# lightdock/lightdock-rust

Measured on AMD Instinct MI355X. Metric: pose-energy evals/sec (DFIRE, 1k4c), higher is better.
Workload: dtype f64; 1 GPU; 1k4c DFIRE pose-energy batch, 8192 poses/GPU/step, 3413 x 3268 atoms, synthetic DCparams; parallelism=swarm-sharded x1, no collectives, nominal_pair_tests_per_pose=11153684

## Files before the change

### lightdock-rust_amd/csrc/kernels/dfire_bm.hip

```cpp
#include "dfire_bm.hpp"

#include <algorithm>
#include <cmath>
#include <cstddef>
#include <cstdlib>
#include <type_traits>

#include "dfire_device.hpp"
#include "dfire_bm_batch.inc"

#if !defined(LD_DIAG_BUILD) && (defined(LD_BM_DIAG_ANM_COST) || defined(LD_BM_DIAG_ANM_LDS) || defined(LD_BM_DIAG_FIRST) || defined(LD_BM_DIAG_NO_ATOMIC) || defined(LD_BM_DIAG_NO_DMA) || defined(LD_BM_DIAG_NO_EXACT) || defined(LD_BM_DIAG_NO_EXACT_ATOMIC) || defined(LD_BM_DIAG_NO_PAIRS) || defined(LD_BM_DIAG_NO_PARTIAL) || defined(LD_BM_DIAG_NO_POSE) || defined(LD_BM_DIAG_NO_TRACKED) || defined(LD_BM_DIAG_ROW_OF_LANE) || defined(LD_BM_DIAG_WAIT) || defined(LD_BM_DIAG_CULL_TIMES) || defined(LD_BM_DIAG_NO_TP_ATOMIC))
#error "LD_BM_DIAG_* needs -DLD_DIAG_BUILD (tools/build_variant.sh)"
#endif

namespace ld {

namespace {

typedef const __attribute__((address_space(4))) BmLaunch BmArgs;
#define LD_BM_ARGS ((BmArgs *)__builtin_amdgcn_kernarg_segment_ptr())

#ifndef LD_BM_CULL_POSES
#define LD_BM_CULL_POSES 8
#endif
// ... 637 lines not shown
        }
        T->job_count[3] = at;
    }
    __syncthreads();
    for (uint32_t base = 0; base < n_jobs; base += 8 * kStep) {
        uint32_t cost[8];
#pragma unroll
        for (int u = 0; u < 8; u++) {
            const uint32_t j = base + (uint32_t)u * kStep + (uint32_t)tid;
            cost[u] = j < n_jobs ? T->job_cost[j] : 0u;
        }
#pragma unroll
        for (int u = 0; u < 8; u++)
            if (cost[u]) T->job_order[atomicAdd(&s_class[class_of(cost[u])], 1u)] = base + (uint32_t)u * kStep + (uint32_t)tid;
    }
}

template <bool ANM>
struct BmWaveSharedT {
    static constexpr int kPart = ANM ? kBmAnmPartEntries : kBmPartEntries;
    unsigned char row_bits[kPart];
    unsigned short items[kPart + 64];
    alignas(16) float modes[ANM ? 2 * kBmModeFloats : 4];
};
template <bool ANM>
struct BmSharedT {
    unsigned char lut[kBmLutBytes];
    unsigned char cube[kBmWaves][kBmCubeBytes];
    BmWaveSharedT<ANM> w[kBmWaves];
};
typedef BmSharedT<false> BmShared;
static_assert(sizeof(BmSharedT<false>) * kBmGroupsPerCu <= 160 * 1024 && sizeof(BmSharedT<true>) * kBmGroupsPerCu <= 160 * 1024, "two workgroups per CU");
static_assert(offsetof(BmShared, cube) + sizeof(unsigned char[kBmWaves][kBmCubeBytes]) < 65536, "cube rows are addressed by instruction offsets");
static_assert(offsetof(BmSharedT<true>, cube) == offsetof(BmShared, cube), "one batch code for both forms");

struct BmWaveCtx {
    size_t tp;
    int ls;
    int RT;
    size_t lo;
};

#ifndef LD_BM_DRAIN_AT
#define LD_BM_DRAIN_AT 256
#endif
#ifndef LD_BM_EXACT_U
#define LD_BM_EXACT_U 4
#endif
constexpr int kBmDrainAt = LD_BM_DRAIN_AT;
__device__ __forceinline__ unsigned long long bm_pair_item(uint32_t row, int la, int ra) {
    return (unsigned long long)row | (unsigned long long)la << 32 | (unsigned long long)ra << 48;
}

__device__ __forceinline__ void bm_exact_pairs(BmArgs *T, unsigned long long *queue, uint32_t n_pairs, int lane) {
#ifdef LD_BM_DIAG_NO_EXACT
    return;
#endif
    __builtin_amdgcn_fence(__ATOMIC_RELEASE, "workgroup");
    constexpr int U = LD_BM_EXACT_U;
    const ExactCtx ex0 = bm_exact_ctx(T, 0);
    const size_t flag_words = (size_t)(T->m.rec_flag_words + T->m.lig.flag_words);
    for (uint32_t base = 0; base < n_pairs; base += 64 * U) {
        unsigned long long item[U];
        bool act[U];
        int la[U], ra[U];
        size_t row[U], pose[U];
#pragma unroll
        for (int u = 0; u < U; u++) {
            const uint32_t k = base + (uint32_t)(u * 64 + lane);
            act[u] = k < n_pairs;
            item[u] = act[u] ? __hip_atomic_load(queue + k, __ATOMIC_RELAXED, __HIP_MEMORY_SCOPE_AGENT) : 0ull;
        }
#pragma unroll
        for (int u = 0; u < U; u++) {
            la[u] = (int)((item[u] >> 32) & 0xffffu);
            ra[u] = (int)(item[u] >> 48);
            act[u] = act[u] && la[u] < T->m.lig.n_real && ra[u] < T->m.rec_n_real;
            row[u] = (size_t)(item[u] & 0xffffffffull);
        }
        typedef double v2d __attribute__((ext_vector_type(2)));
        v2d pq[U][4], lq[U][2], rq[U][2];
#pragma unroll
        for (int u = 0; u < U; u++) {
            const v2d *prow = reinterpret_cast<const v2d *>(T->rt_exact + (act[u] ? row[u] : 0) * 8);
            const v2d *lrow = reinterpret_cast<const v2d *>(T->m.lig_exact + (size_t)(act[u] ? la[u] : 0) * 4);
            const v2d *rrow = reinterpret_cast<const v2d *>(T->m.rec_exact + (size_t)(act[u] ? ra[u] : 0) * 4);
#pragma unroll
            for (int c = 0; c < 4; c++) pq[u][c] = prow[c];
            lq[u][0] = lrow[0]; lq[u][1] = lrow[1];
            rq[u][0] = rrow[0]; rq[u][1] = rrow[1];
        }
        double pr[U][7], lc[U][3], rc[U][3];
        uint32_t lterm[U], rterm[U];
        int32_t rslot[U], lslot[U];
#pragma unroll
        for (int u = 0; u < U; u++) {
            pr[u][0] = pq[u][0].x; pr[u][1] = pq[u][0].y; pr[u][2] = pq[u][1].x; pr[u][3] = pq[u][1].y;
            pr[u][4] = pq[u][2].x; pr[u][5] = pq[u][2].y; pr[u][6] = pq[u][3].x;
            pose[u] = (size_t)__double_as_longlong(pq[u][3].y);
            lc[u][0] = lq[u][0].x; lc[u][1] = lq[u][0].y; lc[u][2] = lq[u][1].x;
            rc[u][0] = rq[u][0].x; rc[u][1] = rq[u][0].y; rc[u][2] = rq[u][1].x;
            const unsigned long long lw = (unsigned long long)__double_as_longlong(lq[u][1].y), rw = (unsigned long long)__double_as_longlong(rq[u][1].y);
            lterm[u] = (uint32_t)lw; lslot[u] = (int32_t)(lw >> 32);
            rterm[u] = (uint32_t)rw; rslot[u] = (int32_t)(rw >> 32);
        }
        bool inside[U];
        uint32_t slot_at[U];
#pragma unroll
        for (int u = 0; u < U; u++) {
            inside[u] = false;
            slot_at[u] = 0u;
            if (!act[u]) continue;
            if (T->exact_pairs) atomicAdd(T->exact_pairs + row[u], 1u);
            const Quat q{pr[u][3], pr[u][4], pr[u][5], pr[u][6]};
            const Quat r = qmul(qmul(q, Quat{0.0, lc[u][0], lc[u][1], lc[u][2]}), qinverse(q));
            double px = r.x + pr[u][0], py = r.y + pr[u][1], pz = r.z + pr[u][2];
            double rx = rc[u][0], ry = rc[u][1], rz = rc[u][2];
            if (T->amp != nullptr) {
                const v2d *amps = reinterpret_cast<const v2d *>(T->amp_exact + row[u] * (2 * kBmMaxModes));
                const v2d *lm = reinterpret_cast<const v2d *>(T->m.lig_modes_exact + (size_t)la[u] * (3 * kBmMaxModes));
                const v2d *rm = reinterpret_cast<const v2d *>(T->m.rec_modes_exact + (size_t)ra[u] * (3 * kBmMaxModes));
#pragma unroll
                for (int k2 = 0; k2 < kBmMaxModes / 2; k2++) {
                    if (2 * k2 < T->m.anm_lig) {
                        const v2d c = amps[kBmMaxModes / 2 + k2], m0 = lm[3 * k2], m1 = lm[3 * k2 + 1], m2 = lm[3 * k2 + 2];
                        px += m0.x * c.x; py += m0.y * c.x; pz += m1.x * c.x;
                        if (2 * k2 + 1 < T->m.anm_lig) { px += m1.y * c.y; py += m2.x * c.y; pz += m2.y * c.y; }
                    }
                    if (2 * k2 < T->m.anm_rec) {
                        const v2d c = amps[k2], m0 = rm[3 * k2], m1 = rm[3 * k2 + 1], m2 = rm[3 * k2 + 2];
                        rx += m0.x * c.x; ry += m0.y * c.x; rz += m1.x * c.x;
                        if (2 * k2 + 1 < T->m.anm_rec) { rx += m1.y * c.y; ry += m2.x * c.y; rz += m2.y * c.y; }
                    }
                }
            }
            const double dx = 2.0 * rx - 2.0 * px, dy = 2.0 * ry - 2.0 * py, dz = 2.0 * rz - 2.0 * pz;
            const double D = dx * dx + dy * dy + dz * dz;
            if (!(D <= kCutScaled)) continue;
            uint32_t bin = 0;
            for (int b = 1; b <= 20; b++) bin += D >= ex0.step4[b] ? 1u : 0u;
            if (D <= ex0.iface_scaled) {
                uint32_t *flags = T->flags + pose[u] * flag_words;
                if (rslot[u] >= 0) atomicOr(&flags[rslot[u] >> 5], 1u << (rslot[u] & 31));
                if (lslot[u] >= 0) atomicOr(&flags[T->m.rec_flag_words + (lslot[u] >> 5)], 1u << (lslot[u] & 31));
            }
            inside[u] = true;
            slot_at[u] = (lterm[u] + rterm[u] + tiled_bin_term(bin)) / 8u;
        }
        double value[U];
#pragma unroll
        for (int u = 0; u < U; u++) value[u] = ex0.table[slot_at[u]];
#pragma unroll
        for (int u = 0; u < U; u++) {
            if (!inside[u]) continue;
            const long long fix = T->count_mode ? 1ll : __double2ll_rn(value[u] * T->m.fix_scale);
#ifndef LD_BM_DIAG_NO_EXACT_ATOMIC
            if (fix != 0) atomicAdd(reinterpret_cast<unsigned long long *>(T->exact_fix + row[u]), (unsigned long long)fix);
#else
            asm volatile("" :: "v"(fix));
#endif
        }
    }
    __builtin_amdgcn_fence(__ATOMIC_ACQ_REL, "workgroup");
}

__device__ __forceinline__ uint32_t bm_cell(float Rs, float Rz, float Ry, float Rx, float l2, float lz, float ly, float lx) {
    float D = Rs - l2;
    D = __builtin_fmaf(Rz, lz, D);
    D = __builtin_fmaf(Ry, ly, D);
    D = __builtin_fmaf(Rx, lx, D);
    uint32_t c;
    asm("v_cvt_u32_f32 %0, %1" : "=v"(c) : "v"(D));
    return c;
}

__device__ __forceinline__ unsigned long long bm_block_item(size_t entry, int a, int b) {
    return (unsigned long long)entry | (unsigned long long)a << 32 | (unsigned long long)b << 35;
}
__device__ __forceinline__ uint32_t bm_recheck(BmArgs *T, const unsigned char *lut, const unsigned long long *blocks, uint32_t n_blocks,
                                            unsigned long long *queue, uint32_t n_pairs, int lane) {
    __builtin_amdgcn_fence(__ATOMIC_RELEASE, "workgroup");
    constexpr float seed = (float)kBmCellZero + 0.5f;
    const int n_rt = T->m.rec_n_tiles;
    for (uint32_t base = 0; base < n_blocks; base += 64) {
    if (n_pairs > (uint32_t)kBmQueuePairs - 4096u - (uint32_t)(8 * kBmPartEntries)) {
        bm_exact_pairs(T, queue, n_pairs, lane);
        n_pairs = 0;
    }
    const bool act = base + (uint32_t)lane < n_blocks;
    const unsigned long long item = act ? __hip_atomic_load(blocks + base + lane, __ATOMIC_RELAXED, __HIP_MEMORY_SCOPE_AGENT) : 0ull;
    const size_t entry = (size_t)(item & 0xffffffffull);
    const int a = (int)((item >> 32) & 7u), b = (int)((item >> 35) & 7u);
    const size_t tp = entry / T->cap;
    const int lt = (int)(tp / (unsigned)n_rt), RT = (int)(tp % (unsigned)n_rt), ls = lt * 8 + a;
    const uint32_t row = act ? T->ent_row[entry] : 0u;
    const float4 *ap = reinterpret_cast<const float4 *>(T->rt) + (size_t)row * 3;
    const float4 a0 = ap[0], a1 = ap[1], a2 = ap[2];
    const TiledBox box = T->m.rec_sub[(size_t)RT * 8 + b];
    const float cbx = 0.5f * (box.lox + box.hix), cby = 0.5f * (box.loy + box.hiy), cbz = 0.5f * (box.loz + box.hiz);
    const Affine A{a0.x, a0.y, a0.z, a0.w - cbx, a1.x, a1.y, a1.z, a1.w - cby, a2.x, a2.y, a2.z, a2.w - cbz};
    const bool anm = T->amp != nullptr;
    float amp_rec[kBmMaxModes], amp_lig[kBmMaxModes];
    bool wild = false;
#pragma unroll
    for (int k = 0; k < kBmMaxModes; k++) amp_rec[k] = amp_lig[k] = 0.f;
    if (anm) {
        const float *am = T->amp + (size_t)row * kBmAmpFloats;
#pragma unroll
        for (int k = 0; k < kBmMaxModes; k++) {
            amp_rec[k] = am[k];
            amp_lig[k] = am[kBmMaxModes + k];
        }
        wild = am[20] != 0.f;
    }
    auto flexed = [&](const float *modes, const float *amps, int atom, int c) {
        const float *m = modes + ((atom >> 1) * 3 + c) * kBmMaxModes * 2 + (atom & 1);
        float d = amps[0] * m[0];
#pragma unroll
        for (int k = 1; k < kBmMaxModes; k++) d = __builtin_fmaf(amps[k], m[2 * k], d);
        return d;
    };
    float lx[8], ly[8], lz[8], l2[8];
#pragma unroll
    for (int i = 0; i < 8; i++) {
        const float4 L = reinterpret_cast<const float4 *>(T->m.lig_local)[ls * 8 + i];
        bm_apply(A, L.x, L.y, L.z, lx[i], ly[i], lz[i]);
        if (anm) {
            const float *lm = T->m.lig_modes_f32 + (size_t)ls * kBmModeFloats;
            lx[i] += flexed(lm, amp_lig, i, 0);
            ly[i] += flexed(lm, amp_lig, i, 1);
            lz[i] += flexed(lm, amp_lig, i, 2);
        }
        l2[i] = __builtin_fmaf(lx[i], lx[i], __builtin_fmaf(ly[i], ly[i], lz[i] * lz[i]));
    }
    const float *rec = reinterpret_cast<const float *>(T->m.rec_pairs + (size_t)RT * 32 + b * 4);
    const uint32_t near_code = T->m.lig_sub_tracked[ls] != 0 || T->m.rec_sub_tracked[RT * 8 + b] != 0 ? bm_code_of_bin(1) : 0xffffffffu;
#pragma unroll 1
    for (int q = 0; q < 4; q++) {
#pragma unroll
        for (int h = 0; h < 2; h++) {
            float x = rec[q * 8 + h] - cbx, y = rec[q * 8 + 2 + h] - cby, z = rec[q * 8 + 4 + h] - cbz;
            if (anm) {
                const float *rm = T->m.rec_modes_f32 + ((size_t)RT * 8 + (size_t)b) * kBmModeFloats;
                x += flexed(rm, amp_rec, 2 * q + h, 0);
                y += flexed(rm, amp_rec, 2 * q + h, 1);
                z += flexed(rm, amp_rec, 2 * q + h, 2);
            }
            const float Rs = __builtin_fmaf(-x, x, __builtin_fmaf(-y, y, __builtin_fmaf(-z, z, seed)));
            const float Rx = x * 2.f, Ry = y * 2.f, Rz = z * 2.f;
#pragma unroll
            for (int i = 0; i < 8; i++) {
                const uint32_t cell = bm_cell(Rs, Rz, Ry, Rx, l2[i], lz[i], ly[i], lx[i]);
                const uint32_t code = lut[cell];
                const bool hit = act && (wild || code == kBmFlagged || (near_code != 0xffffffffu && code <= near_code));
                const unsigned long long m = __builtin_amdgcn_ballot_w64(hit);
                if (hit) {
                    const uint32_t at = n_pairs + __builtin_amdgcn_mbcnt_hi((uint32_t)(m >> 32), __builtin_amdgcn_mbcnt_lo((uint32_t)m, 0u));
                    queue[at] = bm_pair_item(row, ls * 8 + i, RT * 64 + b * 8 + 2 * q + h);
                }
                n_pairs += (uint32_t)__popcll(m);
            }
        }
    }
    }
    return n_pairs;
}

template <bool DEBUG, bool ANM>
__global__ __launch_bounds__(kBmWaves * 64, kBmGroupsPerCu) void dfire_bm_pairs(const BmLaunch launch_arguments) {
    BmArgs *T = LD_BM_ARGS;
    __shared__ __attribute__((aligned(16))) BmSharedT<ANM> S;
    static_assert(offsetof(BmShared, lut) == 0, "the LUT's cell is its LDS address");
    static_assert(kBmWaves * kBmGroupsPerCu == 8, "dfire_bm_batch.inc clobbers v220..v255: 256 VGPRs a wave = two waves per SIMD");
    if ((uint32_t)(uintptr_t)&S != 0u) __builtin_trap();
    const int tid = threadIdx.x, lane = tid & 63;
    const int wave = __builtin_amdgcn_readfirstlane(tid >> 6);
    const int n_rt = T->m.rec_n_tiles;
    if (T->job_count[3] == 0) return;
    {
        const uint8_t *lut = T->count_mode ? T->m.lut_full : T->m.lut;
        for (int i = tid; i < kBmLutBytes / 16; i += kBmWaves * 64) reinterpret_cast<uint4 *>(S.lut)[i] = reinterpret_cast<const uint4 *>(lut)[i];
    }
    BmWaveSharedT<ANM> &WS = S.w[wave];
    __syncthreads();
    const uint32_t n_jobs = T->job_count[3];
    unsigned long long *queue = T->queue + ((size_t)blockIdx.x * kBmWaves + wave) * kBmQueueCap;
    unsigned long long *queue_blocks = queue + kBmQueuePairs;
    uint32_t queued = 0, queued_blocks = 0;
    const unsigned char *table_rows = reinterpret_cast<const unsigned char *>(T->count_mode ? T->m.rows_ones : T->m.rows);
    const unsigned long long dbg_t0 = DEBUG ? __builtin_amdgcn_s_memrealtime() : 0ull;
    unsigned long long dbg_jobs = 0, dbg_batches = 0, dbg_t_batch = 0, dbg_t_drain = 0, dbg_t_scan = 0, dbg_t_block = 0;
    unsigned long long dbg_t_dma = 0, dbg_t_compact = 0, dbg_t_compact_read = 0, dbg_t_chain = 0, dbg_t_wait = 0, dbg_blocks = 0;
    auto now = [] { return DEBUG ? __builtin_amdgcn_s_memrealtime() : 0ull; };

    const uint32_t n_waves = gridDim.x * (uint32_t)kBmWaves;
    bool first_job = true;
    for (;;) {
        const unsigned long long dbg_tj = now();
        uint32_t job = blockIdx.x * (uint32_t)kBmWaves + (uint32_t)wave;
        if (!first_job) {
            if (lane == 0) job = atomicAdd(T->job_next, 1u);
            job = (uint32_t)__builtin_amdgcn_readfirstlane((int)job) + n_waves;
        }
        first_job = false;
        if (job >= n_jobs) break;
        job = T->job_order[job];
        const uint4 rec = reinterpret_cast<const uint4 *>(T->job_rec)[job];
        const size_t tp = (size_t)(uint32_t)__builtin_amdgcn_readfirstlane((int)rec.x);
        const uint32_t lo = (uint32_t)__builtin_amdgcn_readfirstlane((int)rec.y), hi = (uint32_t)__builtin_amdgcn_readfirstlane((int)rec.z);
        const int a = __builtin_amdgcn_readfirstlane((int)rec.w);
        const int lt = (int)(tp / (unsigned)n_rt), RT = (int)(tp % (unsigned)n_rt);
        const int ls = lt * 8 + a;

        const uint32_t roff_all = T->m.rec_rowoff[(size_t)RT * 64 + lane];
        uint32_t any_bits = 0;
        {
            constexpr int kChunks = BmWaveSharedT<ANM>::kPart / 64;
            const unsigned long long *mask_at = T->ent_mask + (tp * T->cap + lo + (size_t)lane);
            unsigned long long m[kChunks];
#pragma unroll
            for (int k = 0; k < kChunks; k++) m[k] = mask_at[k * 64];
            const uint32_t n_mine = hi - lo;
#pragma unroll
            for (int k = 0; k < kChunks; k++) {
                const uint32_t bits = (uint32_t)(k * 64 + lane) < n_mine ? (uint32_t)(m[k] >> (8 * a)) & 0xffu : 0u;
                WS.row_bits[k * 64 + lane] = (unsigned char)bits;
                any_bits |= bits;
            }
        }
#pragma unroll
        for (int off = 32; off > 0; off >>= 1) any_bits |= (uint32_t)__shfl_xor((int)any_bits, off, 64);
        any_bits = (uint32_t)__builtin_amdgcn_readfirstlane((int)any_bits);
        if (any_bits == 0) continue;
        if (DEBUG) dbg_jobs++;

        v2f LocX[4], LocY[4], LocZ[4];
        {
            const float mine = T->m.lig_local[(size_t)(ls * 8 + (lane & 7)) * 4 + (lane < 24 ? lane >> 3 : 0)];
            auto from = [&](int l) { return __int_as_float(__builtin_amdgcn_readlane(__float_as_int(mine), l)); };
#pragma unroll
            for (int p2 = 0; p2 < 4; p2++) {
                LocX[p2] = v2f{from(2 * p2), from(2 * p2 + 1)};
                LocY[p2] = v2f{from(8 + 2 * p2), from(9 + 2 * p2)};
                LocZ[p2] = v2f{from(16 + 2 * p2), from(17 + 2 * p2)};
            }
        }
        if (ANM) {
            __builtin_amdgcn_fence(__ATOMIC_ACQ_REL, "wavefront");
            if (lane < kBmModeFloats / 4) reinterpret_cast<float4 *>(WS.modes)[lane] = reinterpret_cast<const float4 *>(T->m.lig_modes_f32 + (size_t)ls * kBmModeFloats)[lane];
        }
        constexpr int kRowPieces = kBmRowBytes / 16, kDmaRows = 64 / kRowPieces, kDma = (kBmCubeRows + kDmaRows - 1) / kDmaRows;
        static_assert(kRowPieces == 11 && kDmaRows == 5 && kDma == 13, "five rows per copy");
        const bool lig_tracked = T->m.lig_sub_tracked[ls] != 0;
        const uint32_t my_tracked = T->m.rec_sub_tracked[RT * 8 + (lane & 7)];
        const uint32_t lig_rowbase = T->m.lig_rowbase[ls * 8 + (lane & 7)];
        long long *const my_partial = T->ent_partial + ((size_t)blockIdx.x * kBmWaves + wave) * kBmPartEntries;
        const size_t row_base_entry = tp * T->cap + lo;
        const uint32_t *const job_rows = T->ent_row + row_base_entry;
// ... 220 lines not shown
                        const uint32_t lds_at = (uint32_t)(uintptr_t)&WS.items[0];
                        asm volatile(".rept 30\n\t"
                                     "ds_read_b128 v[220:223], %6\n\tds_read_b128 v[224:227], %6 offset:16\n\tds_read_b128 v[228:231], %6 offset:32\n\tds_read_b128 v[232:235], %6 offset:48\n\t"
                                     "s_waitcnt lgkmcnt(0)\n\t"
                                     "v_pk_fma_f32 %0, %4, v[220:221], %0\n\tv_pk_fma_f32 %1, %4, v[222:223], %1\n\tv_pk_fma_f32 %2, %5, v[224:225], %2\n\tv_pk_fma_f32 %3, %5, v[226:227], %3\n\t"
                                     "v_pk_fma_f32 %0, %4, v[228:229], %0\n\tv_pk_fma_f32 %1, %4, v[230:231], %1\n\tv_pk_fma_f32 %2, %5, v[232:233], %2\n\tv_pk_fma_f32 %3, %5, v[234:235], %3\n\t"
                                     ".endr\n\t"
                                     ".rept 9\n\tv_pk_fma_f32 %0, %4, %5, %0\n\tv_pk_fma_f32 %1, %4, %5, %1\n\tv_pk_fma_f32 %2, %4, %5, %2\n\tv_pk_fma_f32 %3, %4, %5, %3\n\t.endr"
                                     : "+v"(t0), "+v"(t1), "+v"(t2), "+v"(t3) : "v"(P.LX[0]), "v"(P.LY[0]), "v"(lds_at)
                                     : "v220", "v221", "v222", "v223", "v224", "v225", "v226", "v227", "v228", "v229", "v230", "v231", "v232", "v233", "v234", "v235", "memory");
                    }
#endif
                    v2f vRs[4], vRz[4], vRy[4], vRx[4];
#pragma unroll
                    for (int q = 0; q < 4; q++) {
                        vRs[q] = Rs[q] + t0 * v2f{0.f, 0.f}; vRz[q] = Rz[q] + t1 * v2f{0.f, 0.f}; vRy[q] = Ry[q] + t2 * v2f{0.f, 0.f}; vRx[q] = Rx[q] + t3 * v2f{0.f, 0.f};
                    }
                    LD_BM_BATCH_ASM_V(acc0, acc1, vRs, vRz, vRy, vRx, P.L2, P.LZ, P.LY, P.LX, kCube);
                }
#elif !defined(LD_BM_DIAG_NO_PAIRS)
                if constexpr (ANM) {
                    LD_BM_BATCH_ASM_V(acc0, acc1, P.fRs, P.fRz, P.fRy, P.fRx, P.L2, P.LZ, P.LY, P.LX, kCube);
                } else {
                    LD_BM_BATCH_ASM(acc0, acc1, Rs, Rz, Ry, Rx, P.L2, P.LZ, P.LY, P.LX, kCube);
                }
#else
                asm volatile("" : "+v"(acc0), "+v"(acc1) : "v"(P.L2[0]), "v"(P.L2[1]), "v"(P.L2[2]), "v"(P.L2[3]), "v"(P.LX[0]), "v"(P.LY[0]), "v"(P.LZ[0]), "s"(Rs[0]), "s"(Rx[3]));
#endif
            };
            auto finish_batch = [&](long long cur_prev, uint32_t cur_item, uint32_t cur_row, bool wild, unsigned long long acc0, unsigned long long acc1, uint32_t done) {
                const int count = n_items - done >= 64u ? 64 : (int)(n_items - done);
                uint32_t invalid;
                asm("v_ashrrev_i32 %0, 31, %1" : "=v"(invalid) : "v"(count - 1 - lane));
                const uint32_t el = cur_item & (uint32_t)kBmEntryMask;
                static_assert(kBmMarkerShift > 33, "the markers sit in the upper word");
                constexpr int kHiShift = kBmMarkerShift - 32;
                const int mark0 = ((int)(uint32_t)(acc0 >> 32) + (1 << (kHiShift - 1))) >> kHiShift, mark1 = ((int)(uint32_t)(acc1 >> 32) + (1 << (kHiShift - 1))) >> kHiShift;
                const unsigned long long marker_bits = (unsigned long long)((uint32_t)(mark0 + mark1) << kHiShift) << 32;
                uint32_t marks = (uint32_t)(mark0 + mark1);
                if constexpr (ANM) marks = wild ? 128u : marks;
                marks &= ~invalid;
                const bool one = marks - 64u < 64u, several = marks >= 128u;
                const unsigned long long m1 = __builtin_amdgcn_ballot_w64(one), m2 = __builtin_amdgcn_ballot_w64(several);
                pending_push = 0xffffffffu;
                if (one) {
                    const int pair = (int)marks - 64;
                    pending_push = queued + __builtin_amdgcn_mbcnt_hi((uint32_t)(m1 >> 32), __builtin_amdgcn_mbcnt_lo((uint32_t)m1, 0u));
                    pending_push_item = bm_pair_item(cur_row, ls * 8 + (pair >> 3), RT * 64 + b * 8 + (pair & 7));
                }
                queued += (uint32_t)__popcll(m1);
                if (__builtin_expect(m2 != 0ull, 0)) {
                    if (several) {
                        pending_push = (uint32_t)kBmQueuePairs + queued_blocks + __builtin_amdgcn_mbcnt_hi((uint32_t)(m2 >> 32), __builtin_amdgcn_mbcnt_lo((uint32_t)m2, 0u));
                        pending_push_item = bm_block_item(row_base_entry + el, a, b);
                    }
                    queued_blocks += (uint32_t)__popcll(m2);
                }
                if constexpr (ANM) pending_val = wild ? cur_prev : (long long)((unsigned long long)cur_prev + acc0 + acc1 - marker_bits);
                else pending_val = (long long)((unsigned long long)cur_prev + acc0 + acc1 - marker_bits);
                pending_item = cur_item | invalid;
                pending_row = cur_row;
            };
            for (uint32_t done = 0; done < n_items; done += 64) {
                if (DEBUG) dbg_batches++;
                const unsigned long long dbg_tb = now();
                if (done == 0) asm volatile("s_waitcnt vmcnt(0)" ::: "memory");
                asm volatile("" :: "v"(next.a0.x), "v"(next.a0.y), "v"(next.a0.z), "v"(next.a0.w), "v"(next.a1.x), "v"(next.a1.y), "v"(next.a1.z), "v"(next.a1.w),
                             "v"(next.a2.x), "v"(next.a2.y), "v"(next.a2.z), "v"(next.a2.w), "v"(next.prev));
                asm volatile("" :: "v"(look_row.row));
                if constexpr (ANM) asm volatile("" :: "v"(next.amp[0].x), "v"(next.amp[1].x), "v"(next.amp[2].x), "v"(next.amp[3].x), "v"(next.amp[4].x), "v"(next.amp[5].x));
                if (DEBUG && done == 0) dbg_t_wait += now() - dbg_tb;
#ifdef LD_BM_DIAG_WAIT
                if (DEBUG) dbg_t_drain += now() - dbg_tb;
#endif
                flush_pending();
                if (done == 0) {
                    long long *row = reinterpret_cast<long long *>(S.cube[wave] + lane * kBmRowBytes);
                    const long long marker = (long long)(64 + lane) << kBmMarkerShift;
                    row[kBmFlagged / 8] = marker;
                    if (tracked) row[0] = row[1] = marker;
                }
                __builtin_amdgcn_fence(__ATOMIC_ACQ_REL, "wavefront");
                Posed P;
                pose_batch(next, P);
                const long long cur_prev = next.prev;
                const uint32_t cur_item = next.item, cur_row = next.row;
                next = issue_loads(look_item, look_row);
                const RowOfItem in_row = read_row(look2_item);
                const uint32_t in_item = read_item(first_of(done + 192u));
                unsigned long long acc0 = 0ull, acc1 = 0ull;
                switch (wave) {
                    case 0: walk_batch(std::integral_constant<int, 0>{}, P, acc0, acc1); break;
                    case 1: walk_batch(std::integral_constant<int, 1>{}, P, acc0, acc1); break;
                    case 2: walk_batch(std::integral_constant<int, 2>{}, P, acc0, acc1); break;
                    default: walk_batch(std::integral_constant<int, 3>{}, P, acc0, acc1); break;
                }
                finish_batch(cur_prev, cur_item, cur_row, P.wild, acc0, acc1, done);
                look_item = look2_item;
                look_row = in_row;
                look2_item = in_item;
                if (DEBUG) dbg_t_batch += now() - dbg_tb;
#ifdef LD_BM_DIAG_FIRST
                if (DEBUG && done == 0) dbg_t_drain += now() - dbg_tb;
#endif
            }
            flush_pending();
        }
        if (queued_blocks >= 64u) {
            const unsigned long long td = now();
            queued = bm_recheck(T, S.lut, queue_blocks, queued_blocks, queue, queued, lane);
            queued_blocks = 0;
            if (DEBUG) dbg_t_drain += now() - td;
        }
        if (queued >= (uint32_t)kBmDrainAt) {
            const unsigned long long td = now();
            bm_exact_pairs(T, queue, queued, lane);
            queued = 0;
            if (DEBUG) dbg_t_drain += now() - td;
        }
    }
    {
        const unsigned long long td = now();
        if (queued_blocks) queued = bm_recheck(T, S.lut, queue_blocks, queued_blocks, queue, queued, lane);
        if (queued) bm_exact_pairs(T, queue, queued, lane);
        if (DEBUG) dbg_t_drain += now() - td;
    }
#ifndef LD_BM_DIAG_CULL_TIMES
    if (DEBUG && T->debug != nullptr && lane == 0) {
        unsigned long long *d = T->debug + ((size_t)blockIdx.x * kBmWaves + wave) * kBmDebugWords;
        d[0] = dbg_t0;
        d[1] = __builtin_amdgcn_s_memrealtime();
        d[2] = dbg_jobs;
        d[3] = dbg_batches;
        d[4] = dbg_t_batch;
        d[5] = dbg_t_drain;
        d[6] = dbg_t_block;
        d[7] = dbg_t_scan;
        d[8] = dbg_t_dma;
        d[9] = dbg_t_compact;
        d[10] = dbg_t_chain;
        d[11] = dbg_t_wait;
        d[12] = dbg_blocks;
        d[13] = dbg_t_compact_read;
    }
#endif
}

__global__ __launch_bounds__(256) void dfire_bm_gather(const BmLaunch launch_arguments) {
    BmArgs *T = LD_BM_ARGS;
    const int n_lt = T->m.lig.n_tiles;
    const size_t n_rows = bm_rows(T);
    const int sub = (int)threadIdx.x & 7;
    const size_t rows_per_trip = (size_t)gridDim.x * 32;
    for (size_t first = (size_t)blockIdx.x * 32; first < n_rows; first += rows_per_trip) {
        const size_t row = first + threadIdx.x / 8;
        const bool valid = row < n_rows;
        const long long pp = valid ? bm_pose_of(T, row) : -1;
        double units = 0.0;
        uint32_t tested = 0;
        if (pp >= 0)
            for (int lt = sub; lt < n_lt; lt += 8) {
                units += (double)T->tile_sum[(size_t)lt * T->cap + row];
                if (T->count_mode && T->tile_tested) tested += T->tile_tested[row * (size_t)n_lt + lt];
            }
#pragma unroll
        for (int off = 4; off > 0; off >>= 1) {
            units += __shfl_xor(units, off, 64);
            tested += (uint32_t)__shfl_xor((int)tested, off, 64);
        }
        if (pp < 0 || sub != 0) continue;
        const size_t pose = (size_t)pp;
        units += (double)T->exact_fix[row];
        if (T->count_mode) {
            T->count_partial[pose] = (uint32_t)units;
            if (T->tested_partial) T->tested_partial[pose] = tested;
            if (T->exact_partial) T->exact_partial[pose] = T->exact_pairs[row];
        } else {
            T->partial[2 * pose] = units * (1.0 / T->m.fix_scale);
            T->partial[2 * pose + 1] = 0.0;
        }
    }
}

}

size_t bm_pairs_lds_bytes() { return sizeof(BmShared); }

hipError_t launch_bm_pose(const BmLaunch &t, hipStream_t stream) {
    if (t.n_poses == 0) return hipSuccess;
    hipLaunchKernelGGL(dfire_bm_pose, dim3((unsigned)std::min<size_t>((t.n_poses + 255) / 256, 2048)), dim3(256), 0, stream, t);
    return hipGetLastError();
}

hipError_t launch_bm_cull(const BmLaunch &t, hipStream_t stream) {
    if (t.n_poses == 0) return hipSuccess;
    if (t.m.rec_n_tiles > 1024 || t.n_poses > kBmMaxPassPoses) return hipErrorInvalidValue;
// ... 57 lines not shown
```

### lightdock-rust_amd/csrc/kernels/dfire_bm.hpp

```cpp
#pragma once

#include <hip/hip_runtime.h>

#include <cstddef>
#include <cstdint>

#include "dfire_tiled.hpp"

namespace ld {

constexpr int kBmCells = 16;
constexpr double kBmKappa = 8.0;
constexpr int kBmCutCell = 900 * kBmCells;
constexpr int kBmLutBytes = 14592;
constexpr float kBmCellMax = 14591.0f;
constexpr int kBmCellZero = 14583;
constexpr int kBmRowSlots = 22;
constexpr int kBmRowBytes = kBmRowSlots * 8;
constexpr uint32_t kBmMissCode = 8 * 20;
constexpr uint32_t kBmFlagged = 8 * 21;
__host__ __device__ inline uint32_t bm_code_of_bin(uint32_t bin) { return 8 * bin; }
constexpr int kBmMarkerShift = 51;
constexpr int kBmJobRows = 8;
constexpr int kBmPartEntries = 1792;
constexpr int kBmDebugWords = 14;
constexpr int kBmEntryMask = 0x7ff;
constexpr int kBmPassQuantum = 1024;
constexpr int kBmOpsFloats = 36;
constexpr int kBmMaxModes = 10;
constexpr int kBmModeFloats = 8 * 3 * kBmMaxModes;
constexpr int kBmAmpFloats = 24;
constexpr int kBmAnmPartEntries = 1024;
constexpr float kBmWildUnits = 128.0f;
constexpr int kBmCubeRows = 64;
constexpr int kBmCubeBytes = kBmCubeRows * kBmRowBytes;
constexpr int kBmTypes = 170;
constexpr int kBmWaves = 4;
constexpr int kBmGroupsPerCu = 2;
constexpr int kBmWavesPerCu = kBmWaves * kBmGroupsPerCu;
constexpr int kBmQueuePairs = 8 * kBmPartEntries + 4096 + 512;
constexpr int kBmQueueCap = kBmQueuePairs + 8 * kBmPartEntries + 64;
constexpr double kBmFixLimit = 1024.0;
constexpr int kBmCounters = 8;
constexpr int kBmCullQueueWords = 256;
constexpr int kBmCostClasses = 80;
#ifndef LD_BM_CULL_WAVES
#define LD_BM_CULL_WAVES 4
#endif
constexpr int kBmCullWaves = LD_BM_CULL_WAVES;
constexpr size_t kBmLdsPerCu = 160 * 1024;
__host__ __device__ inline size_t bm_cull_lds_for(int n_rt, int hit_tiles) {
    const int hit_cap = hit_tiles * n_rt > 192 ? hit_tiles * n_rt : 192;
    return (size_t)n_rt * 9 * 32 + (size_t)kBmCullWaves * (((size_t)hit_cap * 14 + (size_t)n_rt * 8 + 15) / 16 * 16);
}
__host__ __device__ inline int bm_cull_hit_tiles(int n_rt) {
    int k = 4;
    while (k > 1 && bm_cull_lds_for(n_rt, k) + 1024 > kBmLdsPerCu) k--;
    return k;
}
__host__ __device__ inline int bm_cull_hit_cap(int n_rt) { const int k = bm_cull_hit_tiles(n_rt); return k * n_rt > 192 ? k * n_rt : 192; }
__host__ __device__ inline size_t bm_cull_wave_lds(int n_rt) { return ((size_t)bm_cull_hit_cap(n_rt) * 14 + (size_t)n_rt * 8 + 15) / 16 * 16; }
__host__ __device__ inline size_t bm_cull_lds_bytes(int n_rt) { return bm_cull_lds_for(n_rt, bm_cull_hit_tiles(n_rt)); }
constexpr float kBmBoxCutUnits2 = 14400.0f * 1.00005f;
constexpr size_t kBmMaxPassPoses = 262144;

struct BmModel {
    int rec_n_real = 0, rec_n_tiles = 0;
    const PackedRecPair *rec_pairs = nullptr;
    const TiledBox *rec_sub = nullptr;
    const TiledBox *rec_tile = nullptr;
    const uint32_t *rec_rowoff = nullptr;
    const float *rec_ops = nullptr;
    const double *rec_x = nullptr, *rec_y = nullptr, *rec_z = nullptr;
    const uint32_t *rec_tindex = nullptr;
    const int32_t *rec_slot = nullptr;
    int rec_flag_words = 0;
    int anm_rec = 0, anm_lig = 0;
    const float *rec_modes_f32 = nullptr;
// ... 181 lines not shown
```

### lightdock-rust_amd/csrc/scorer.cpp

```cpp
#include "scorer.hpp"

#include <algorithm>
#include <cmath>
#include <cstdio>
#include <cstdlib>
#include <cstring>
#include <limits>

#include "host/spatial_order.hpp"

#if defined(__SANITIZE_ADDRESS__)
#include <sanitizer/asan_interface.h>
#else
#define ASAN_POISON_MEMORY_REGION(addr, size) ((void)(addr), (void)(size))
#define ASAN_UNPOISON_MEMORY_REGION(addr, size) ((void)(addr), (void)(size))
#endif

namespace ld {

DeviceArena::~DeviceArena() {
    for (void *p : blocks_) (void)hipFree(p);
}
void *DeviceArena::alloc_bytes(size_t bytes) {
    void *p = nullptr;
// ... 1126 lines not shown
    t.m = model_;
    t.poses = d_poses;
    t.stride = stride;
    t.active = d_list ? nullptr : d_active;
    t.pose_list = d_list;
    t.pose_count = d_list ? d_count : nullptr;
    t.cap = s.cap;
    t.pairs_groups = n_cus_;
    t.flags = out.flags;
    t.partial = out.partial;
    t.count_partial = out.count_partial;
    t.tested_partial = out.tested_partial;
    t.exact_partial = out.exact_partial;
    if (s.anm) t.part_cap = (uint32_t)kBmAnmPartEntries;
    if (const char *e = std::getenv("LIGHTDOCK_BM_PART_CAP")) {
        const long v = std::atol(e);
        if (v >= 64 && v % 64 == 0 && (uint32_t)v <= (s.anm ? (uint32_t)kBmAnmPartEntries : (uint32_t)kBmPartEntries)) t.part_cap = (uint32_t)v;
    }
    if (dbg) {
        ws_.point(t, layout, 0);
        hip_check(hipMemsetAsync(t.debug, 0, layout.region[kBmRegDebug].bytes, stream), "hipMemsetAsync debug");
    }
    const bool two_lanes = s.sets == 2;
    if (two_lanes) {
        hip_check(hipEventRecord(fork_, stream), "hipEventRecord");
        hip_check(hipStreamWaitEvent(aux_stream_, fork_, 0), "hipStreamWaitEvent");
    }
    int lane = 0;
    for (size_t off = 0; off < n; off += s.cap, lane ^= 1) {
        hipStream_t st = lane && two_lanes ? aux_stream_ : stream;
        t.first = off;
        t.n_poses = std::min(s.cap, n - off);
        ws_.point(t, layout, two_lanes ? (size_t)lane : 0);
        uint32_t *const tile_tested = t.tile_tested, *const exact_pairs = t.exact_pairs;
        for (int mode = counts ? 1 : 0; mode >= 0; mode--) {
            t.count_mode = mode;
            t.tile_tested = mode ? tile_tested : nullptr;
            t.exact_pairs = mode ? exact_pairs : nullptr;
            hip_check(launch_bm_pose(t, st), "launch dfire_bm_pose");
            hip_check(launch_bm_cull(t, st), "launch dfire_bm_cull");
            hip_check(launch_bm_pairs(t, st), "launch dfire_bm_pairs");
            hip_check(launch_bm_gather(t, st), "launch dfire_bm_gather");
        }
    }
    if (two_lanes) {
        hip_check(hipEventRecord(join_, aux_stream_), "hipEventRecord");
        hip_check(hipStreamWaitEvent(stream, join_, 0), "hipStreamWaitEvent");
    }
    if (dbg) {
        hip_check(hipStreamSynchronize(stream), "hipStreamSynchronize");
        std::vector<unsigned long long> h(s.waves * kBmDebugWords);
        hip_check(hipMemcpy(h.data(), t.debug, h.size() * 8, hipMemcpyDeviceToHost), "D2H debug");
        if (FILE *f = std::fopen(dbg, "w")) {
            for (size_t i = 0; i < h.size(); i += kBmDebugWords)
                for (int k = 0; k < kBmDebugWords; k++) std::fprintf(f, k + 1 < kBmDebugWords ? "%llu " : "%llu\n", h[i + (size_t)k]);
            std::fclose(f);
        }
    }
}

Scorer::~Scorer() {
    for (auto &e : events_) {
        (void)hipEventDestroy(e.first);
        (void)hipEventDestroy(e.second);
    }
    if (own_stream_) {
        (void)hipStreamSynchronize(own_stream_);
        (void)hipStreamDestroy(own_stream_);
    }
}

uint64_t Scorer::workspace_generation() const {
    uint64_t g = 0;
    for (const DeviceBuffer *b : {&ws_partial_, &ws_flags_, &ws_counts_, &ws_tested_, &ws_exact_}) g += b->generation;
    return g + (bm_ ? bm_->generation() : 0) + (packed_ ? packed_->generation() : 0);
}

size_t Scorer::partials_per_pose() const {
    return bm_ ? 1 : packed_ ? packed_->partials_per_pose() : all_pairs_->partials_per_pose();
}

void Scorer::reserve_workspace(size_t n_poses, bool counts) {
    const size_t words = (size_t)(rec_.flag_words + lig_.flag_words);
    const size_t chunks = partials_per_pose();
    ws_partial_.reserve(n_poses * chunks * 2 * sizeof(double));
    ws_flags_.reserve(std::max<size_t>(n_poses * words * sizeof(uint32_t), 16));
    if (counts) {
        ws_counts_.reserve(n_poses * chunks * sizeof(uint32_t));
        ws_tested_.reserve(n_poses * chunks * sizeof(uint32_t));
        ws_exact_.reserve(n_poses * chunks * sizeof(uint32_t));
    }
    if (bm_) bm_->reserve(n_poses, counts);
}

void Scorer::energy_batch_device(size_t n, const double *d_poses, size_t stride, const uint8_t *d_active,
                                 double *d_energies, uint32_t *d_pair_counts, const uint32_t *d_list, const uint32_t *d_count) {
    if (n == 0) return;
    if (!d_poses || !d_energies) throw Error(LD_ERR_INVALID, "energy_batch: null pose/energy buffer");
    if (stride < pose_len()) throw Error(LD_ERR_INVALID, "energy_batch: stride shorter than a pose row");
    if (d_list && (!d_active || !d_count)) throw Error(LD_ERR_INVALID, "energy_batch: a pose list needs its device-side count and the matching active mask");
    const size_t max_n = packed_ ? packed_->max_batch() : n;
    if (n > max_n) {
        for (size_t off = 0; off < n; off += max_n)
            energy_batch_device(std::min(max_n, n - off), d_poses + off * stride, stride, d_active ? d_active + off : nullptr,
                                d_energies + off, d_pair_counts ? d_pair_counts + off : nullptr);
        return;
    }
    reserve_workspace(n, d_pair_counts != nullptr);
// ... 137 lines not shown
```

Measured before the change: 8.073 million evals/s.

## Pack row into block items, bitmask recheck hits with DPP prefix scan, unify drain loop

```diff
diff --git a/lightdock-rust_amd/csrc/kernels/dfire_bm.hip b/lightdock-rust_amd/csrc/kernels/dfire_bm.hip
--- a/lightdock-rust_amd/csrc/kernels/dfire_bm.hip
+++ b/lightdock-rust_amd/csrc/kernels/dfire_bm.hip
@@ -713,10 +713,33 @@
     return (unsigned long long)row | (unsigned long long)la << 32 | (unsigned long long)ra << 48;
 }
 
-__device__ __forceinline__ void bm_exact_pairs(BmArgs *T, unsigned long long *queue, uint32_t n_pairs, int lane) {
+struct BmDrainDebug {
+    unsigned long long t_items = 0;
+    unsigned long long t_rows = 0;
+    unsigned long long t_arith = 0;
+    unsigned long long t_table = 0;
+    unsigned long long t_atomics = 0;
+    unsigned long long t_first = 0;
+    unsigned long long drains = 0, trips = 0, pairs = 0, max_trips = 0;
+    unsigned long long t_recheck = 0, rounds = 0, block_items = 0;
+};
+
+template <bool DEBUG, bool ANM>
+__device__ __forceinline__ void bm_exact_pairs(BmArgs *T, unsigned long long *queue, uint32_t n_pairs, int lane, BmDrainDebug &dbg) {
 #ifdef LD_BM_DIAG_NO_EXACT
     return;
 #endif
+    auto now = [] { return DEBUG ? __builtin_amdgcn_s_memrealtime() : 0ull; };
+    auto arrived = [] { if (DEBUG) asm volatile("s_waitcnt vmcnt(0)" ::: "memory"); };
+    unsigned long long dbg_t = now(), dbg_trips = 0;
+    const unsigned long long dbg_first0 = dbg_t;
+    auto lap = [&](unsigned long long &phase) {
+        if (DEBUG) {
+            const unsigned long long t = now();
+            phase += t - dbg_t;
+            dbg_t = t;
+        }
+    };
     __builtin_amdgcn_fence(__ATOMIC_RELEASE, "workgroup");
     constexpr int U = LD_BM_EXACT_U;
     const ExactCtx ex0 = bm_exact_ctx(T, 0);
@@ -732,6 +755,8 @@
             act[u] = k < n_pairs;
             item[u] = act[u] ? __hip_atomic_load(queue + k, __ATOMIC_RELAXED, __HIP_MEMORY_SCOPE_AGENT) : 0ull;
         }
+        arrived();
+        lap(dbg.t_items);
 #pragma unroll
         for (int u = 0; u < U; u++) {
             la[u] = (int)((item[u] >> 32) & 0xffffu);
@@ -751,6 +776,12 @@
             lq[u][0] = lrow[0]; lq[u][1] = lrow[1];
             rq[u][0] = rrow[0]; rq[u][1] = rrow[1];
         }
+        if (DEBUG) {
+#pragma unroll
+            for (int u = 0; u < U; u++) dbg.pairs += (unsigned long long)__popcll(__builtin_amdgcn_ballot_w64(act[u]));
+        }
+        arrived();
+        lap(dbg.t_rows);
         double pr[U][7], lc[U][3], rc[U][3];
         uint32_t lterm[U], rterm[U];
         int32_t rslot[U], lslot[U];
@@ -777,7 +808,7 @@
             const Quat r = qmul(qmul(q, Quat{0.0, lc[u][0], lc[u][1], lc[u][2]}), qinverse(q));
             double px = r.x + pr[u][0], py = r.y + pr[u][1], pz = r.z + pr[u][2];
             double rx = rc[u][0], ry = rc[u][1], rz = rc[u][2];
-            if (T->amp != nullptr) {
+            if (ANM && T->amp != nullptr) {
                 const v2d *amps = reinterpret_cast<const v2d *>(T->amp_exact + row[u] * (2 * kBmMaxModes));
                 const v2d *lm = reinterpret_cast<const v2d *>(T->m.lig_modes_exact + (size_t)la[u] * (3 * kBmMaxModes));
                 const v2d *rm = reinterpret_cast<const v2d *>(T->m.rec_modes_exact + (size_t)ra[u] * (3 * kBmMaxModes));
@@ -808,9 +839,12 @@
             inside[u] = true;
             slot_at[u] = (lterm[u] + rterm[u] + tiled_bin_term(bin)) / 8u;
         }
+        lap(dbg.t_arith);
         double value[U];
 #pragma unroll
         for (int u = 0; u < U; u++) value[u] = ex0.table[slot_at[u]];
+        arrived();
+        lap(dbg.t_table);
 #pragma unroll
         for (int u = 0; u < U; u++) {
             if (!inside[u]) continue;
@@ -821,8 +855,18 @@
             asm volatile("" :: "v"(fix));
 #endif
         }
+        if (DEBUG) {
+            lap(dbg.t_atomics);
+            if (dbg_trips++ == 0) dbg.t_first += dbg_t - dbg_first0;
+        }
     }
     __builtin_amdgcn_fence(__ATOMIC_ACQ_REL, "workgroup");
+    if (DEBUG) {
+        lap(dbg.t_atomics);
+        dbg.drains++;
+        dbg.trips += dbg_trips;
+        dbg.max_trips = dbg_trips > dbg.max_trips ? dbg_trips : dbg.max_trips;
+    }
 }
 
 __device__ __forceinline__ uint32_t bm_cell(float Rs, float Rz, float Ry, float Rx, float l2, float lz, float ly, float lx) {
@@ -835,32 +879,34 @@
     return c;
 }
 
-__device__ __forceinline__ unsigned long long bm_block_item(size_t entry, int a, int b) {
-    return (unsigned long long)entry | (unsigned long long)a << 32 | (unsigned long long)b << 35;
-}
-__device__ __forceinline__ uint32_t bm_recheck(BmArgs *T, const unsigned char *lut, const unsigned long long *blocks, uint32_t n_blocks,
-                                            unsigned long long *queue, uint32_t n_pairs, int lane) {
+static_assert(kBmMaxPassPoses <= (size_t)1 << 26, "a block item keeps the row of the pass in its upper 26 bits");
+__device__ __forceinline__ unsigned long long bm_block_item(size_t entry, int a, int b, uint32_t row) {
+    return (unsigned long long)entry | (unsigned long long)a << 32 | (unsigned long long)b << 35 | (unsigned long long)row << 38;
+}
+template <bool DEBUG, bool ANM>
+__device__ __forceinline__ uint32_t bm_recheck(BmArgs *T, const unsigned char *lut, const unsigned long long *blocks, uint32_t &n_blocks,
+                                            unsigned long long *queue, uint32_t n_pairs, int lane, BmDrainDebug &dbg) {
+    const unsigned long long dbg_t = DEBUG ? __builtin_amdgcn_s_memrealtime() : 0ull;
+    if (DEBUG) dbg.block_items += n_blocks;
     __builtin_amdgcn_fence(__ATOMIC_RELEASE, "workgroup");
     constexpr float seed = (float)kBmCellZero + 0.5f;
     const int n_rt = T->m.rec_n_tiles;
-    for (uint32_t base = 0; base < n_blocks; base += 64) {
-    if (n_pairs > (uint32_t)kBmQueuePairs - 4096u - (uint32_t)(8 * kBmPartEntries)) {
-        bm_exact_pairs(T, queue, n_pairs, lane);
-        n_pairs = 0;
-    }
+    while (n_blocks != 0u && n_pairs <= (uint32_t)kBmQueuePairs - 4096u - (uint32_t)(8 * kBmPartEntries)) {
+    const uint32_t base = (n_blocks - 1u) & ~63u;
+    if (DEBUG) dbg.rounds++;
     const bool act = base + (uint32_t)lane < n_blocks;
     const unsigned long long item = act ? __hip_atomic_load(blocks + base + lane, __ATOMIC_RELAXED, __HIP_MEMORY_SCOPE_AGENT) : 0ull;
-    const size_t entry = (size_t)(item & 0xffffffffull);
+    const uint32_t entry = (uint32_t)item;
     const int a = (int)((item >> 32) & 7u), b = (int)((item >> 35) & 7u);
-    const size_t tp = entry / T->cap;
+    const uint32_t tp = entry / (uint32_t)T->cap;
     const int lt = (int)(tp / (unsigned)n_rt), RT = (int)(tp % (unsigned)n_rt), ls = lt * 8 + a;
-    const uint32_t row = act ? T->ent_row[entry] : 0u;
+    const uint32_t row = (uint32_t)(item >> 38);
     const float4 *ap = reinterpret_cast<const float4 *>(T->rt) + (size_t)row * 3;
     const float4 a0 = ap[0], a1 = ap[1], a2 = ap[2];
     const TiledBox box = T->m.rec_sub[(size_t)RT * 8 + b];
     const float cbx = 0.5f * (box.lox + box.hix), cby = 0.5f * (box.loy + box.hiy), cbz = 0.5f * (box.loz + box.hiz);
     const Affine A{a0.x, a0.y, a0.z, a0.w - cbx, a1.x, a1.y, a1.z, a1.w - cby, a2.x, a2.y, a2.z, a2.w - cbz};
-    const bool anm = T->amp != nullptr;
+    const bool anm = ANM && T->amp != nullptr;
     float amp_rec[kBmMaxModes], amp_lig[kBmMaxModes];
     bool wild = false;
 #pragma unroll
@@ -895,9 +941,12 @@
         l2[i] = __builtin_fmaf(lx[i], lx[i], __builtin_fmaf(ly[i], ly[i], lz[i] * lz[i]));
     }
     const float *rec = reinterpret_cast<const float *>(T->m.rec_pairs + (size_t)RT * 32 + b * 4);
-    const uint32_t near_code = T->m.lig_sub_tracked[ls] != 0 || T->m.rec_sub_tracked[RT * 8 + b] != 0 ? bm_code_of_bin(1) : 0xffffffffu;
+    const int near_code = T->m.lig_sub_tracked[ls] != 0 || T->m.rec_sub_tracked[RT * 8 + b] != 0 ? (int)bm_code_of_bin(1) : -1;
+    const uint32_t wild_sign = wild ? 0x80000000u : 0u;
+    unsigned long long hits = 0ull;
 #pragma unroll 1
     for (int q = 0; q < 4; q++) {
+        uint32_t hits_q = 0u;
 #pragma unroll
         for (int h = 0; h < 2; h++) {
             float x = rec[q * 8 + h] - cbx, y = rec[q * 8 + 2 + h] - cby, z = rec[q * 8 + 4 + h] - cbz;
@@ -913,16 +962,35 @@
             for (int i = 0; i < 8; i++) {
                 const uint32_t cell = bm_cell(Rs, Rz, Ry, Rx, l2[i], lz[i], ly[i], lx[i]);
                 const uint32_t code = lut[cell];
-                const bool hit = act && (wild || code == kBmFlagged || (near_code != 0xffffffffu && code <= near_code));
-                const unsigned long long m = __builtin_amdgcn_ballot_w64(hit);
-                if (hit) {
-                    const uint32_t at = n_pairs + __builtin_amdgcn_mbcnt_hi((uint32_t)(m >> 32), __builtin_amdgcn_mbcnt_lo((uint32_t)m, 0u));
-                    queue[at] = bm_pair_item(row, ls * 8 + i, RT * 64 + b * 8 + 2 * q + h);
-                }
-                n_pairs += (uint32_t)__popcll(m);
-            }
-        }
-    }
+                const uint32_t sign = ((code ^ kBmFlagged) - 1u) | (code - (uint32_t)near_code - 1u) | wild_sign;
+                hits_q = hits_q << 1 | sign >> 31;
+            }
+        }
+        hits |= (unsigned long long)hits_q << (16 * q);
+    }
+    if (!act) hits = 0ull;
+    const uint32_t mine = (uint32_t)__popcll(hits);
+    uint32_t upto = mine;
+    upto += (uint32_t)__builtin_amdgcn_update_dpp(0, (int)upto, 0x111, 0xf, 0xf, false);
+    upto += (uint32_t)__builtin_amdgcn_update_dpp(0, (int)upto, 0x112, 0xf, 0xf, false);
+    upto += (uint32_t)__builtin_amdgcn_update_dpp(0, (int)upto, 0x114, 0xf, 0xf, false);
+    upto += (uint32_t)__builtin_amdgcn_update_dpp(0, (int)upto, 0x118, 0xf, 0xf, false);
+    upto += (uint32_t)__builtin_amdgcn_update_dpp(0, (int)upto, 0x142, 0xa, 0xf, false);
+    upto += (uint32_t)__builtin_amdgcn_update_dpp(0, (int)upto, 0x143, 0xc, 0xf, false);
+    uint32_t at = n_pairs + upto - mine;
+    n_pairs += (uint32_t)__builtin_amdgcn_readlane((int)upto, 63);
+    while (__builtin_amdgcn_ballot_w64(hits != 0ull) != 0ull) {
+        if (hits != 0ull) {
+            const int k = __builtin_ctzll(hits) ^ 15;
+            hits &= hits - 1ull;
+            queue[at++] = bm_pair_item(row, ls * 8 + (k & 7), RT * 64 + b * 8 + (k >> 3));
+        }
+    }
+    n_blocks = base;
+    }
+    if (DEBUG) {
+        dbg.block_items -= n_blocks;
+        dbg.t_recheck += __builtin_amdgcn_s_memrealtime() - dbg_t;
     }
     return n_pairs;
 }
@@ -944,7 +1012,7 @@
     }
     BmWaveSharedT<ANM> &WS = S.w[wave];
     __syncthreads();
-    const uint32_t n_jobs = T->job_count[3];
+    uint32_t n_jobs = T->job_count[3];
     unsigned long long *queue = T->queue + ((size_t)blockIdx.x * kBmWaves + wave) * kBmQueueCap;
     unsigned long long *queue_blocks = queue + kBmQueuePairs;
     uint32_t queued = 0, queued_blocks = 0;
@@ -953,10 +1021,25 @@
     unsigned long long dbg_jobs = 0, dbg_batches = 0, dbg_t_batch = 0, dbg_t_drain = 0, dbg_t_scan = 0, dbg_t_block = 0;
     unsigned long long dbg_t_dma = 0, dbg_t_compact = 0, dbg_t_compact_read = 0, dbg_t_chain = 0, dbg_t_wait = 0, dbg_blocks = 0;
     auto now = [] { return DEBUG ? __builtin_amdgcn_s_memrealtime() : 0ull; };
+    BmDrainDebug dbg_drain;
 
     const uint32_t n_waves = gridDim.x * (uint32_t)kBmWaves;
     bool first_job = true;
     for (;;) {
+        const bool last = n_jobs == 0u;
+        if (queued >= (uint32_t)kBmDrainAt || queued_blocks >= 64u || (last && (queued | queued_blocks) != 0u)) {
+            const unsigned long long td = now();
+            BmArgs *Tx = T;
+            asm volatile("" : "+s"(Tx));
+            auto blocks_due = [&] { return queued_blocks >= 64u || (last && queued_blocks != 0u); };
+            do {
+                if (blocks_due()) queued = bm_recheck<DEBUG, ANM>(Tx, S.lut, queue_blocks, queued_blocks, queue, queued, lane, dbg_drain);
+                if (queued != 0u) bm_exact_pairs<DEBUG, ANM>(Tx, queue, queued, lane, dbg_drain);
+                queued = 0;
+            } while (blocks_due());
+            if (DEBUG) dbg_t_drain += now() - td;
+        }
+        if (last) break;
         const unsigned long long dbg_tj = now();
         uint32_t job = blockIdx.x * (uint32_t)kBmWaves + (uint32_t)wave;
         if (!first_job) {
@@ -964,7 +1047,10 @@
             job = (uint32_t)__builtin_amdgcn_readfirstlane((int)job) + n_waves;
         }
         first_job = false;
-        if (job >= n_jobs) break;
+        if (job >= n_jobs) {
+            n_jobs = 0u;
+            continue;
+        }
         job = T->job_order[job];
         const uint4 rec = reinterpret_cast<const uint4 *>(T->job_rec)[job];
         const size_t tp = (size_t)(uint32_t)__builtin_amdgcn_readfirstlane((int)rec.x);
@@ -1291,7 +1377,7 @@
                 if (__builtin_expect(m2 != 0ull, 0)) {
                     if (several) {
                         pending_push = (uint32_t)kBmQueuePairs + queued_blocks + __builtin_amdgcn_mbcnt_hi((uint32_t)(m2 >> 32), __builtin_amdgcn_mbcnt_lo((uint32_t)m2, 0u));
-                        pending_push_item = bm_block_item(row_base_entry + el, a, b);
+                        pending_push_item = bm_block_item(row_base_entry + el, a, b, cur_row);
                     }
                     queued_blocks += (uint32_t)__popcll(m2);
                 }
@@ -1345,42 +1431,25 @@
             }
             flush_pending();
         }
-        if (queued_blocks >= 64u) {
-            const unsigned long long td = now();
-            queued = bm_recheck(T, S.lut, queue_blocks, queued_blocks, queue, queued, lane);
-            queued_blocks = 0;
-            if (DEBUG) dbg_t_drain += now() - td;
-        }
-        if (queued >= (uint32_t)kBmDrainAt) {
-            const unsigned long long td = now();
-            bm_exact_pairs(T, queue, queued, lane);
-            queued = 0;
-            if (DEBUG) dbg_t_drain += now() - td;
-        }
-    }
-    {
-        const unsigned long long td = now();
-        if (queued_blocks) queued = bm_recheck(T, S.lut, queue_blocks, queued_blocks, queue, queued, lane);
-        if (queued) bm_exact_pairs(T, queue, queued, lane);
-        if (DEBUG) dbg_t_drain += now() - td;
     }
 #ifndef LD_BM_DIAG_CULL_TIMES
     if (DEBUG && T->debug != nullptr && lane == 0) {
         unsigned long long *d = T->debug + ((size_t)blockIdx.x * kBmWaves + wave) * kBmDebugWords;
+        auto both = [](unsigned long long low, unsigned long long high) { return (low & 0xffffffffull) | high << 32; };
         d[0] = dbg_t0;
         d[1] = __builtin_amdgcn_s_memrealtime();
-        d[2] = dbg_jobs;
-        d[3] = dbg_batches;
-        d[4] = dbg_t_batch;
-        d[5] = dbg_t_drain;
-        d[6] = dbg_t_block;
-        d[7] = dbg_t_scan;
-        d[8] = dbg_t_dma;
-        d[9] = dbg_t_compact;
-        d[10] = dbg_t_chain;
-        d[11] = dbg_t_wait;
-        d[12] = dbg_blocks;
-        d[13] = dbg_t_compact_read;
+        d[2] = both(dbg_jobs, dbg_drain.t_items);
+        d[3] = both(dbg_batches, dbg_drain.t_rows);
+        d[4] = both(dbg_t_batch, dbg_drain.t_arith);
+        d[5] = both(dbg_t_drain, dbg_drain.t_table);
+        d[6] = both(dbg_t_block, dbg_drain.t_atomics);
+        d[7] = both(dbg_t_scan, dbg_drain.t_first);
+        d[8] = both(dbg_t_dma, dbg_drain.drains);
+        d[9] = both(dbg_t_compact, dbg_drain.trips);
+        d[10] = both(dbg_t_chain, dbg_drain.pairs);
+        d[11] = both(dbg_t_wait, dbg_drain.t_recheck);
+        d[12] = both(dbg_blocks, dbg_drain.block_items);
+        d[13] = both(dbg_t_compact_read, dbg_drain.rounds << 8 | (dbg_drain.max_trips & 0xffull));
     }
 #endif
 }
diff --git a/lightdock-rust_amd/csrc/kernels/dfire_bm.hpp b/lightdock-rust_amd/csrc/kernels/dfire_bm.hpp
--- a/lightdock-rust_amd/csrc/kernels/dfire_bm.hpp
+++ b/lightdock-rust_amd/csrc/kernels/dfire_bm.hpp
@@ -24,6 +24,17 @@
 constexpr int kBmJobRows = 8;
 constexpr int kBmPartEntries = 1792;
 constexpr int kBmDebugWords = 14;
+constexpr int kBmDebugColumns = 27;
+inline void bm_debug_columns(const unsigned long long *record, unsigned long long *columns) {
+    columns[0] = record[0];
+    columns[1] = record[1];
+    for (int k = 2; k < kBmDebugWords; k++) columns[k] = record[k] & 0xffffffffull;
+    for (int k = 0; k < 9; k++) columns[14 + k] = record[2 + k] >> 32;
+    columns[23] = (record[13] >> 32) & 0xffull;
+    columns[24] = record[11] >> 32;
+    columns[25] = record[13] >> 40;
+    columns[26] = record[12] >> 32;
+}
 constexpr int kBmEntryMask = 0x7ff;
 constexpr int kBmPassQuantum = 1024;
 constexpr int kBmOpsFloats = 36;
diff --git a/lightdock-rust_amd/csrc/scorer.cpp b/lightdock-rust_amd/csrc/scorer.cpp
--- a/lightdock-rust_amd/csrc/scorer.cpp
+++ b/lightdock-rust_amd/csrc/scorer.cpp
@@ -1202,8 +1202,11 @@
         std::vector<unsigned long long> h(s.waves * kBmDebugWords);
         hip_check(hipMemcpy(h.data(), t.debug, h.size() * 8, hipMemcpyDeviceToHost), "D2H debug");
         if (FILE *f = std::fopen(dbg, "w")) {
-            for (size_t i = 0; i < h.size(); i += kBmDebugWords)
-                for (int k = 0; k < kBmDebugWords; k++) std::fprintf(f, k + 1 < kBmDebugWords ? "%llu " : "%llu\n", h[i + (size_t)k]);
+            for (size_t i = 0; i < h.size(); i += kBmDebugWords) {
+                unsigned long long line[kBmDebugColumns];
+                bm_debug_columns(h.data() + i, line);
+                for (int k = 0; k < kBmDebugColumns; k++) std::fprintf(f, k + 1 < kBmDebugColumns ? "%llu " : "%llu\n", line[k]);
+            }
             std::fclose(f);
         }
     }
```

Result: faster. 8.162 million evals/s (median of 6 runs) (+1.1%).
